# soedinglab/plass

Measured on AMD Instinct MI355X. Metric: read-overlaps/s per assembly iteration, higher is better.
Workload: dtype u8/u64 (integer hash, byte compare; f32 ratios)

## Files before the change

### plass_amd/csrc/assemble.hip

```cpp
#include "common.hpp"
#include "device_utils.hpp"
#include "posterior_class.hpp"
#include "ref_rules.hpp"
#include "asm_rules.hpp"
#include "host_util.hpp"
#include <algorithm>
#include <memory>
#include <cstring>

namespace plasship {

struct Item {
    uint32_t target; int32_t score; uint32_t alnLength; float seqId;
    int32_t qStart, qEnd; uint32_t qLen; int32_t dbStart, dbEnd; uint32_t dbLen;
    uint32_t state;
    uint32_t pad;
};

struct AsmArgs {
    SeqView s;
    const uint64_t *qoff; const AlnRec *recs;
    Item *items;
    const uint64_t *arenaOff;
    const uint32_t *leftCap;
    char *arena;
    uint32_t *flags;
    uint32_t *newLen;
    uint64_t *newStart;
    const signed char *mat;
    double lambda, logK, ln2;
    float seqIdThr; uint64_t maxSeqLen; int rescoreMode;
    uint32_t ownLaneMin;
    unsigned long long *stats;
    uint32_t *bigList; uint32_t nBig;
    const uint32_t *bigCount;
    uint32_t *overList; uint32_t *overCount;
    uint32_t queueCap;
    uint32_t *dbgRounds; uint32_t *dbgCycles;
    uint32_t *midList; uint32_t nMid;
    uint32_t *mid32List; uint32_t nMid32;
    uint32_t *smallList; uint32_t nSmall;
    uint32_t *narrowList; uint32_t nNarrow;
    uint32_t *heap;
    const uint32_t *ambKeys; const uint8_t *ambVals; uint32_t ambMask;
    uint32_t *needKeys; uint32_t *needCount; uint32_t needCap;
    uint32_t *redoList; uint32_t *redoCount;
    const uint32_t *queryList; uint32_t nQueryList;
    uint8_t *cmpCache;
    SeqView aa; char *aaArena; const uint64_t *aaArenaOff; const uint32_t *aaLeftCap; uint32_t *aaNewLen; uint64_t *aaNewStart;
};

__device__ __forceinline__ float seqIdThroughText(float f) {
    if (f == 1.0f) return 1.0f;
    const int t = (int) (f * 1000);
    int zeros = 0;
    if ((double) f < 0.10) zeros++;
    if ((double) f < 0.01) zeros++;
    int digits = 1; for (int x = t; x >= 10; x /= 10) digits++;
    double den = 1.0; for (int i = 0; i < digits + zeros; i++) den *= 10.0;
    return (float) ((double) t / den);
}

template <int G> __device__ __forceinline__ void copyBytesG(char *dst, const char *src, unsigned n, int gl) {
    for (unsigned i = 8u * (unsigned) gl; i < n; i += 8u * G) {
        const uint64_t w = loadU64Unaligned(src + i);
        if (i + 8 <= n) storeU64Unaligned(dst + i, w);
        else storeTail(dst + i, w, n - i);
    }
}
__device__ __forceinline__ void stageScoreTable(signed char *smat, const signed char *__restrict__ mat, int nThreads) {
    for (int i = threadIdx.x; i < 123 * 123; i += nThreads) smat[i] = i ? mat[i] : (signed char) 0;
}
__device__ __forceinline__ uint64_t byteRangeMask(int lo, int hi) {
    const uint64_t belowHi = hi >= 8 ? ~0ULL : (hi <= 0 ? 0ULL : ((1ULL << (8 * hi)) - 1ULL));
    const uint64_t belowLo = lo >= 8 ? ~0ULL : (lo <= 0 ? 0ULL : ((1ULL << (8 * lo)) - 1ULL));
    return belowHi & ~belowLo;
}
__device__ __forceinline__ int zeroBytesMasked(uint64_t x, uint64_t mask) {
    const uint64_t lo7 = 0x7F7F7F7F7F7F7F7FULL;
    return __popcll(~(((x & lo7) + lo7) | x | lo7) & mask);
}
template <int G> __device__ __forceinline__ void scoreColumnsG(const char *q, const char *t, unsigned len, const signed char *smat, int gl,
                                                               unsigned &first, unsigned &last, int &s, int &ids) {
    const unsigned p0 = 8u * (unsigned) gl;
    uint64_t qw = 0, tw = 0;
    if (p0 < len) { qw = loadU64Unaligned(q + p0); tw = loadU64Unaligned(t + p0); }
    const char q0 = q[0], t0 = t[0], qe = q[len - 1], te = t[len - 1];
    first = (q0 == '*' || t0 == '*') ? 1u : 0u;
    last = len - 1;
    if (last > 0 && (qe == '*' || te == '*')) last--;
    for (unsigned p = p0; p < len; p += 8u * G) {
        if (p != p0) { qw = loadU64Unaligned(q + p); tw = loadU64Unaligned(t + p); }
        const int lo = (int) first - (int) p, hi = (int) last - (int) p;
        uint64_t qv = qw, tv = tw;
        if (lo <= 0 && hi >= 8) ids += zeroBytesMasked(qw ^ tw, ~0ULL);
        else {
            const uint64_t m = byteRangeMask(lo, hi + 1);
            ids += zeroBytesMasked(qw ^ tw, byteRangeMask(lo, hi));
            qv = qw & m; tv = tw & m;
        }
#pragma unroll
        for (unsigned j = 0; j < 8; j++) {
// ... 911 lines not shown
        }
    }
    nExt = waveReduceSumU64(nExt); nResc = waveReduceSumU64(nResc); nRescRes = waveReduceSumU64(nRescRes); nAln = waveReduceSumU64(nAln); nQRes = waveReduceSumU64(nQRes);
    if (laneId() == 0) {
        if (nExt) atomicAdd(&a.stats[0], nExt); if (nResc) atomicAdd(&a.stats[1], nResc); if (nRescRes) atomicAdd(&a.stats[2], nRescRes);
        if (nAln) { atomicAdd(&a.stats[3], nAln); atomicAdd(&a.stats[4], nQRes); atomicAdd(&a.stats[5], nRescRes); }
    }
}

template <int G> __device__ __forceinline__ int groupSum(int v) {
    v = rowSum<(G < 16 ? G : 16)>(v);
#pragma unroll
    for (int o = 16; o < G; o <<= 1) v += __shfl_xor(v, o, G);
    return v;
}
template <int G> __device__ __forceinline__ unsigned long long groupMax(unsigned long long v) {
    v = rowMax<(G < 16 ? G : 16)>(v);
#pragma unroll
    for (int o = 16; o < G; o <<= 1) { const unsigned long long ok = __shfl_xor(v, o, G); v = (ok > v) ? ok : v; }
    return v;
}
template <int G> __device__ __forceinline__ uint32_t groupRank(uint32_t mine) {
    if (G == 8) return rowCountLess8(mine);
    uint32_t r = rowCountLess16(mine, mine, false);
#pragma unroll
    for (int o = 16; o < G; o += 16) r += rowCountLess16((uint32_t) __shfl_xor((int) mine, o, G), mine, true);
    return r;
}
template <int G> __device__ __forceinline__ unsigned long long groupBallot(bool p) {
    const unsigned long long m = __ballot(p);
    if (G == 64) return m;
    return (m >> ((laneId() / G) * G)) & ((1ULL << G) - 1ULL);
}

template <int G>
__device__ __forceinline__ Rescored rescoreOnDiagonalG(const char *q, unsigned qLen, const char *t, unsigned tLen, int diagonal,
                                                       const signed char *smat, int gl) {
    Rescored r; r.startPos = -1; r.endPos = -1; r.score = 0; r.diagonalLen = 0; r.idExcl = 0;
    const unsigned dist = (unsigned) abs(diagonal);
    unsigned qo, to, len;
    if (diagonal >= 0 && dist < qLen) { qo = dist; to = 0; len = min(tLen, qLen - dist); }
    else if (diagonal < 0 && dist < tLen) { qo = 0; to = dist; len = min(tLen - dist, qLen); }
    else return r;
    r.diagonalLen = len;
    if (len == 0) return r;
    unsigned first, last;
    int s = 0, ids = 0;
    scoreColumnsG<G>(q + qo, t + to, len, smat, gl, first, last, s, ids);
    s = groupSum<G>(s); ids = groupSum<G>(ids);
    r.score = (unsigned) max(s, 0); r.startPos = (int) first; r.endPos = (int) last; r.idExcl = ids;
    return r;
}

constexpr int ASM8_WPE = 5;
template <int G, int WPE>
__global__ __launch_bounds__(256) __attribute__((amdgpu_waves_per_eu(WPE, WPE))) void assembleGroupKernel(AsmArgs a) {
    __shared__ signed char smat[123 * 123 + 7];
    stageScoreTable(smat, a.mat, 256);
    __syncthreads();
    const int gl = threadIdx.x & (G - 1);
    const uint32_t groupsTotal = gridDim.x * (256 / G);
    const uint32_t nWork = (G == 64) ? a.nMid : ((G == 32) ? a.nMid32 : ((G == 16) ? a.nSmall : a.nNarrow));
    unsigned long long nExt = 0, nResc = 0, nRescRes = 0, nAln = 0, nQRes = 0;
    const uint32_t *workList = (G == 64) ? a.midList : ((G == 32) ? a.mid32List : ((G == 16) ? a.smallList : a.narrowList));
    auto loadWord = [&](uint32_t pid) -> uint64_t {
        uint64_t v = 0;
        if (pid != 0xFFFFFFFFu) {
            if (gl == 0) v = a.qoff[pid]; else if (gl == 1) v = a.qoff[pid + 1]; else if (gl == 2) v = a.arenaOff[pid]; else if (gl == 3) v = a.s.offLen[pid]; else if (gl == 4) v = a.leftCap[pid];
        }
        return v;
    };
    uint32_t w = blockIdx.x * (256 / G) + threadIdx.x / G;
    uint32_t idNext = (w < nWork) ? workList[w] : 0xFFFFFFFFu;
    uint64_t wordNext = loadWord(idNext);
    uint32_t idAhead = (w + groupsTotal < nWork) ? workList[w + groupsTotal] : 0xFFFFFFFFu;
    for (; w < nWork; w += groupsTotal) {
        const uint32_t id = idNext;
        const uint64_t h0 = __shfl(wordNext, 0, G), h1 = __shfl(wordNext, 1, G), aoff = __shfl(wordNext, 2, G), qOffLen = __shfl(wordNext, 3, G), qLeftCap = __shfl(wordNext, 4, G);
        idNext = idAhead; wordNext = loadWord(idNext);
        idAhead = (w + 2u * groupsTotal < nWork) ? workList[w + 2u * groupsTotal] : 0xFFFFFFFFu;
        const uint32_t h = (uint32_t) (h1 - h0);
        const char *orig = a.s.data + (qOffLen >> 24);
        unsigned querySeqLen = (unsigned) ((uint32_t) qOffLen & 0xFFFFFFu);
        if (gl == 0) { nAln += h; nQRes += querySeqLen; }
        uint32_t xTarget = 0xFFFFFFFFu, xAlnLen = 0, xQLen = 0, xDbLen = 0, xState = 2, xTLen = 0; uint64_t xTOff = 0;
        int xScore = 0, xQStart = 0, xQEnd = 0, xDbStart = 0, xDbEnd = 0;
        if ((uint32_t) gl < h) {
            const AlnRec r = a.recs[h0 + gl];
            xTarget = r.target;
            xAlnLen = (uint32_t) alnLengthOf(r.qStart, r.qEnd, r.dbStart, r.dbEnd);
            xScore = scorePerCol100(rawScoreOfBits(r.bitScore, a.ln2, a.logK, a.lambda), xAlnLen);
            xQStart = r.qStart; xQEnd = r.qEnd; xQLen = (uint32_t) r.qLen; xDbStart = r.dbStart; xDbEnd = r.dbEnd; xDbLen = (uint32_t) r.dbLen;
            xState = (xTarget == id || !r.accepted) ? 2u : 0u;
            const bool branchType = ((xDbStart == 0 && xDbEnd != (int) xDbLen - 1) || (xQStart == 0 && xQEnd != (int) xQLen - 1)) && !(xDbStart == 0 && xQStart == 0);
            if (xState == 0 && branchType) { xTOff = seqOff(a.s, xTarget); xTLen = seqLen(a.s, xTarget); }
        }
        const uint32_t tRank = groupRank<G>(xTarget);
        char *buf = a.arena + aoff;
        uint64_t curStart = qLeftCap;
        copyBytesG<G>(buf + curStart, orig, querySeqLen, gl);
        uint64_t curLen = querySeqLen;
        bool couldExtend = false;
        uint32_t inQueue = (uint32_t) __popcll(groupBallot<G>(xState == 0));
        while (inQueue > 0) {
            unsigned leftOff = 0, rightOff = 0;
            bool brokeOut = false;
            if (xState == 1) xState = 2;
            unsigned long long key = 0;
            bool rType = false, lType = false, rBranch = false, lBranch = false;
            unsigned fragR = 0;
            if (xState == 0) {
                key = ((unsigned long long) ((uint32_t) xScore ^ 0x80000000u) << 32) | ((unsigned long long) xAlnLen << 6) | (unsigned long long) (63u - tRank);
                if (isBranchType(xQStart, xQEnd, xQLen, xDbStart, xDbEnd, xDbLen)) {
                    if (xDbStart == 0) { rBranch = true; fragR = rightFragLen(xTLen, xDbEnd); rType = canExtendRight(fragR, xQEnd, querySeqLen); }
                    else if (xQStart == 0) { lBranch = true; lType = canExtendLeft(xDbStart, xDbEnd, xTLen); }
                }
            }
            const unsigned long long bestR = groupMax<G>(rType ? key : 0ULL), bestL = groupMax<G>(lType ? key : 0ULL);
            const bool rFirst = bestR != 0 && bestR > bestL;
            const bool isR = rType && key == bestR, isL = lType && key == bestL;
            auto extendRight = [&]() {
                const int bi = __ffsll((long long) groupBallot<G>(isR)) - 1;
                const char *tSeq = a.s.data + __shfl(xTOff, bi, G);
                const uint32_t bTarget = __shfl(xTarget, bi, G);
                const unsigned fragLen = __shfl(fragR, bi, G), dbEnd = (unsigned) __shfl(xDbEnd, bi, G);
                copyBytesG<G>(buf + curStart + curLen, tSeq + dbEnd + 1, fragLen, gl);
                curLen += fragLen; rightOff += fragLen;
                if (gl == 0) atomicOr(&a.flags[bTarget], 0x80u);
            };
            if (rFirst) extendRight();
            if (bestL != 0) {
                const int bi = __ffsll((long long) groupBallot<G>(isL)) - 1;
                const unsigned fragLen = (unsigned) __shfl(xDbStart, bi, G);
                if (curLen + fragLen >= a.maxSeqLen) brokeOut = true;
                else {
                    const char *tSeq = a.s.data + __shfl(xTOff, bi, G);
                    const uint32_t bTarget = __shfl(xTarget, bi, G);
                    curStart -= fragLen;
                    copyBytesG<G>(buf + curStart, tSeq, fragLen, gl);
                    curLen += fragLen; leftOff += fragLen;
                    if (gl == 0) atomicOr(&a.flags[bTarget], 0x80u);
                }
            }
            if (bestR != 0 && !rFirst && !brokeOut) extendRight();
            if (xState == 0 && (!brokeOut || key >= bestL)) {
                uint32_t st = 2;
                if (!(isR && (rFirst || !brokeOut)) && !isL) {
                    if (rBranch) { if (deferredRight(fragR, xQEnd, querySeqLen, rightOff)) st = 1; }
                    else if (lBranch) { if (deferredLeft(xDbStart, xDbEnd, xTLen, leftOff)) st = 1; }
                }
                xState = st;
            }
            inQueue = (uint32_t) __popcll(groupBallot<G>(xState == 0));
            if (leftOff > 0 || rightOff > 0) couldExtend = true;
            if (brokeOut && inQueue > 0) break;
            querySeqLen = (unsigned) curLen;
            const char *qs = buf + curStart;
            unsigned long long deferred = groupBallot<G>(xState == 1);
            if (deferred) waveMemSync();
            if (G >= 32 && (uint32_t) __popcll(deferred) >= a.ownLaneMin) {
                if (xState == 1) {
                    const char *tSeq = a.s.data + xTOff;
                    const int diag = (int) ((unsigned) xQStart + leftOff) - xDbStart;
                    const DiagSpan sp = diagonalSpan(diag, querySeqLen, xTLen);
                    unsigned first = 0, last = 0; int sc = 0, ids = 0; int startPos = -1, endPos = -1;
                    if (sp.hit && sp.len > 0) { scoreColumnsSerial(qs + sp.qo, tSeq + sp.to, sp.len, smat, first, last, sc, ids); startPos = (int) first; endPos = (int) last; }
                    const unsigned score = (unsigned) max(sc, 0);
                    nResc += 1; nRescRes += sp.len;
                    const AlnCoords c = alnOnDiagonal(diag, startPos, endPos);
                    xQLen = querySeqLen; xDbLen = xTLen; xAlnLen = sp.len; xScore = scorePerCol100(score, sp.len);
                    xQStart = c.qStart; xQEnd = c.qEnd; xDbStart = c.dbStart; xDbEnd = c.dbEnd;
                    xState = (rescoredSeqId(ids, c.qStart, c.qEnd) >= a.seqIdThr) ? 0u : 2u;
                }
                deferred = 0;
            }
            while (deferred) {
                const int dl = __ffsll((long long) deferred) - 1;
                deferred &= deferred - 1;
                const int dqs = __shfl(xQStart, dl, G), dds = __shfl(xDbStart, dl, G);
                const char *tSeq = a.s.data + __shfl(xTOff, dl, G);
                const unsigned tLen = __shfl(xTLen, dl, G);
                const int diag = (int) ((unsigned) dqs + leftOff) - dds;
                const Rescored rs = rescoreOnDiagonalG<G>(qs, querySeqLen, tSeq, tLen, diag, smat, gl);
                nResc += (gl == 0); nRescRes += (gl == 0) ? rs.diagonalLen : 0;
                const AlnCoords c = alnOnDiagonal(diag, rs.startPos, rs.endPos);
                const float seqId = rescoredSeqId(rs.idExcl, c.qStart, c.qEnd);
                if (gl == dl) {
                    xQLen = querySeqLen; xDbLen = tLen; xAlnLen = rs.diagonalLen; xScore = scorePerCol100(rs.score, rs.diagonalLen);
                    xQStart = c.qStart; xQEnd = c.qEnd; xDbStart = c.dbStart; xDbEnd = c.dbEnd;
                    xState = (seqId >= a.seqIdThr) ? 0u : 2u;
                }
            }
            inQueue = (uint32_t) __popcll(groupBallot<G>(xState == 0));
        }
        if (couldExtend) {
            if (gl == 0) { atomicOr(&a.flags[id], 0x20u); a.newLen[id] = (uint32_t) curLen; a.newStart[id] = aoff + curStart; nExt++; }
        }
    }
    nExt = waveReduceSumU64(nExt); nResc = waveReduceSumU64(nResc); nRescRes = waveReduceSumU64(nRescRes); nAln = waveReduceSumU64(nAln); nQRes = waveReduceSumU64(nQRes);
    if (laneId() == 0) {
        if (nExt) atomicAdd(&a.stats[0], nExt); if (nResc) atomicAdd(&a.stats[1], nResc); if (nRescRes) atomicAdd(&a.stats[2], nRescRes);
        const int tier = (G <= 16) ? 0 : 1;
        if (nAln) { atomicAdd(&a.stats[3 + 3 * tier], nAln); atomicAdd(&a.stats[4 + 3 * tier], nQRes); atomicAdd(&a.stats[5 + 3 * tier], nRescRes); }
    }
}

__global__ __launch_bounds__(256) void arenaSumKernel(const AlnRec *__restrict__ recs, uint64_t nAln, uint64_t maxSeqLen, unsigned long long *__restrict__ qSum,
                                                      unsigned long long *__restrict__ qSumAa, uint32_t *__restrict__ qCan, int mirror) {
    const int lane = laneId();
    for (uint64_t i = (uint64_t) blockIdx.x * blockDim.x + threadIdx.x; i < nAln; i += (uint64_t) gridDim.x * blockDim.x) {
        const AlnRec r = recs[i];
        const uint32_t id = r.query;
        uint32_t add = 0, addAa = 0; bool can = false;
        if (r.target != id && r.accepted) {
            add = (uint32_t) r.dbLen; addAa = (uint32_t) r.dbLen / 3 + 2;
            AlnCoords c; c.qStart = r.qStart; c.qEnd = r.qEnd; c.dbStart = r.dbStart; c.dbEnd = r.dbEnd;
            if (mirror && c.qStart > c.qEnd) c = mirrorReverseHit(r.qStart, r.qEnd, r.dbStart, r.dbEnd, (unsigned) r.dbLen);
            if (isBranchType(c.qStart, c.qEnd, (unsigned) r.qLen, c.dbStart, c.dbEnd, (unsigned) r.dbLen)) {
                if (c.dbStart == 0) can = canExtendRight(rightFragLen((unsigned) r.dbLen, c.dbEnd), c.qEnd, (unsigned) r.qLen);
                else if (c.qStart == 0) can = canExtendLeft(c.dbStart, c.dbEnd, (unsigned) r.dbLen) && ((uint64_t) r.qLen + (uint64_t) c.dbStart < maxSeqLen);
            }
        }
        const unsigned long long act = __ballot(1);
        const uint32_t prevId = (uint32_t) __shfl_up((int) id, 1, 64);
        const bool head = lane == 0 || prevId != id;
        const unsigned long long heads = __ballot(head), cans = __ballot(can);
        const int segStart = 63 - __clzll((long long) (heads & (lane == 63 ? ~0ULL : ((2ULL << lane) - 1ULL))));
        const unsigned long long later = lane == 63 ? 0ULL : (heads & ~((2ULL << lane) - 1ULL));
// ... 462 lines not shown
        (guided && (dAaLens.alloc((M + 1) * 8) != hipSuccess || dAaStart.alloc((M + 2) * 8) != hipSuccess))) { setError("plasship_assemble: out of device memory"); return PLASSHIP_ERR_DEVICE; }
    if (M) {
        const unsigned gridM = (unsigned) std::min<uint64_t>((M + 255) / 256, 8192);
        hipLaunchKernelGGL(extLensKernel, dim3(gridM), dim3(256), 0, st, gMeta.as<ExtMeta>(), M, dLens.as<uint64_t>(), guided ? dAaLens.as<uint64_t>() : (uint64_t *) nullptr);
        if (exclusiveScanU64(st, dLens.as<uint64_t>(), dStart.as<uint64_t>(), M, dTmp2.p, tmp2Bytes) ||
            (guided && exclusiveScanU64(st, dAaLens.as<uint64_t>(), dAaStart.as<uint64_t>(), M, dTmp2.p, tmp2Bytes))) { setError("plasship_assemble: scan failed"); return PLASSHIP_ERR_DEVICE; }
        hipLaunchKernelGGL(extMergeKernel, dim3(gridM), dim3(256), 0, st, gMeta.as<ExtMeta>(), M, dStart.as<uint64_t>(), guided ? dAaStart.as<uint64_t>() : (const uint64_t *) nullptr,
                           dFlags, dNewLen, dNewStart, dAaNewLen, dAaNewStart);
    }
    PH_TRACE(st, "assemble: merged the extended sequences");
    if (!keepTarget) {
        DevBuf gFlags;
        rc = commAllgathervBytes(ctx, dFlags, (uint64_t) N * 4, gFlags, rb); if (rc) return rc;
        if (N) hipLaunchKernelGGL(orFlagsKernel, dim3(gridN), dim3(256), 0, st, gFlags.as<uint32_t>(), N, W, dFlags);
        PH_CHECK(plasship::streamSync(st));
    }
    PH_CHECK(plasship::streamSync(st));
    PH_CHECK(hipGetLastError());
    return PLASSHIP_OK;
}

static bool asmHistOn() { return getenv("PLASSHIP_DEBUG_ASMHIST") != nullptr; }
static int asmHistRecord(hipStream_t st, uint32_t N, const uint64_t *dQoff, const uint32_t *dBigList, uint32_t nBig, const uint32_t *dRounds, const uint32_t *dCycles,
                         uint32_t cap, const uint32_t *tierQueries) {
    static int call = 0;
    std::vector<uint32_t> ids(nBig), rounds(N), cycles(N);
    std::vector<uint64_t> qoff((size_t) N + 1);
    if (nBig) PH_COPY_SYNC(st, ids.data(), dBigList, (size_t) nBig * 4, hipMemcpyDeviceToHost);
    PH_COPY_SYNC(st, qoff.data(), dQoff, ((size_t) N + 1) * 8, hipMemcpyDeviceToHost);
    PH_COPY_SYNC(st, rounds.data(), dRounds, (size_t) N * 4, hipMemcpyDeviceToHost);
    PH_COPY_SYNC(st, cycles.data(), dCycles, (size_t) N * 4, hipMemcpyDeviceToHost);
    constexpr int NH = 5, NR = 8;
    uint64_t hq[NH] = {}, hx[NH] = {}, hr[NH] = {}, hc[NH] = {}, hm[NH] = {}, rq[NR] = {}, ct = 0, over = 0, maxH = 0;
    for (uint32_t w = 0; w < nBig; w++) {
        const uint32_t id = ids[w], h = (uint32_t) (qoff[id + 1] - qoff[id]), r = rounds[id] & 0x7FFFFFFFu;
        int b = 0; while (b < NH - 1 && h > (128u << b)) b++;
        int k = 0; if (r) { k = 1; uint32_t e = 1; while (k < NR - 1 && r > e) { e <<= 1; k++; } }
        hq[b]++; hx[b] += rounds[id] >> 31; hr[b] += r; hm[b] = std::max<uint64_t>(hm[b], r); hc[b] += cycles[id]; ct += cycles[id];
        rq[k]++; over += h > cap; maxH = std::max<uint64_t>(maxH, h);
    }
    std::string s = "asmHist call " + std::to_string(call++) + " big queries " + std::to_string(nBig) + " (max h " + std::to_string(maxH) + ", over cap " +
                    std::to_string(cap) + ": " + std::to_string(over) + ") | h bins <=128,<=256,<=512,<=1024,more: queries/extended/mean rounds/max rounds/% ticks";
    for (int b = 0; b < NH; b++) {
        char t[96];
        snprintf(t, sizeof(t), " [%llu %llu %.2f %llu %.1f%%]", (unsigned long long) hq[b], (unsigned long long) hx[b], hq[b] ? (double) hr[b] / hq[b] : 0.0,
                 (unsigned long long) hm[b], ct ? 100.0 * hc[b] / ct : 0.0);
        s += t;
    }
    s += " | rounds 0,1,2,<=4,<=8,<=16,<=32,more:";
    for (int k = 0; k < NR; k++) s += " " + std::to_string(rq[k]);
    s += " | tier queries <=8,<=16,<=32,<=64,more:";
    for (int t = 0; t < 5; t++) s += " " + std::to_string(tierQueries[t]);
    fprintf(stderr, "%s\n", s.c_str());
    return PLASSHIP_OK;
}

static int assembleImpl(plasship_ctx *ctx, const plasship_seqdb *db, const plasship_seqdb *aaDb, const plasship_alns *al,
                        const plasship_assemble_params *par, plasship_seqdb **out, plasship_seqdb **outAa, plasship_assemble_stats *stats) {
    const bool guided = aaDb != nullptr;
    const bool nucl = db->dbtype == PLASSHIP_DBTYPE_NUCLEOTIDES;
    if (!nucl && db->dbtype != PLASSHIP_DBTYPE_AMINO_ACIDS) { setError("plasship_assemble: the sequence DB is neither amino acids nor nucleotides"); return PLASSHIP_ERR_ARG; }
    if (par->rescore_mode != 3) { setError("plasship_assemble: only --rescore-mode 3"); return PLASSHIP_ERR_UNSUPPORTED; }
    if (al->nQueries != db->n) { setError("plasship_assemble: alignment list does not belong to the DB"); return PLASSHIP_ERR_ARG; }
    PH_ENTER(ctx);
    hipStream_t st = ctx->stream;
    const uint32_t N = (uint32_t) db->n;
    if (nucl) { const int rcS = finishSelfAlns(ctx, al); if (rcS) return rcS; }
    const uint64_t nLines = al->nSlots;
    DevBuf dLeftCap, dBytes, dArenaOff, dTmp, dItems, dFlags, dNewLen, dNewStart, dMat, dStats, dArena;
    const size_t tmpBytes = exclusiveScanTmpBytes((size_t) N + 2);
    if (dLeftCap.alloc(((size_t) N + 1) * 4) != hipSuccess || dBytes.alloc(((size_t) N + 1) * 8) != hipSuccess || dArenaOff.alloc(((size_t) N + 2) * 8) != hipSuccess ||
        dTmp.alloc(tmpBytes) != hipSuccess || dItems.alloc(std::max<uint64_t>(nLines, 1) * sizeof(Item)) != hipSuccess || dFlags.alloc(((size_t) N + 1) * 4) != hipSuccess ||
        dNewLen.alloc(((size_t) N + 1) * 4) != hipSuccess || dNewStart.alloc(((size_t) N + 1) * 8) != hipSuccess || dMat.alloc(123 * 123) != hipSuccess || dStats.alloc(128) != hipSuccess) {
        setError("plasship_assemble: out of device memory"); return PLASSHIP_ERR_DEVICE;
    }
    PH_CHECK(hipMemsetAsync(dFlags.p, 0, ((size_t) N + 1) * 4, st));
    PH_CHECK(hipMemsetAsync(dNewLen.p, 0, ((size_t) N + 1) * 4, st));
    PH_CHECK(hipMemsetAsync(dStats.p, 0, 128, st));
    PH_CHECK(hipMemcpyAsync(dMat.p, asciiSubMat(nucl), 123 * 123, hipMemcpyHostToDevice, st));
    { const int rcOL = ensureOffLen(ctx, db); if (rcOL) return rcOL; }
    const SeqView sv = db->view();
    PH_CHECK(hipEventRecord(ctx->ev[0], st));
    const uint32_t nTiles = (uint32_t) (((size_t) N + SCAN_TILE - 1) / SCAN_TILE);
    DevBuf dBigList, dMidList, dMid32List, dSmallList, dNarrowList, dTierOf, dTierPart, dAaLeftCap, dAaBytes, dAaArenaOff, dAaArena, dAaNewLen, dAaNewStart;
    if (guided && (dAaLeftCap.alloc(((size_t) N + 1) * 4) != hipSuccess || dAaBytes.alloc(((size_t) N + 1) * 8) != hipSuccess || dAaArenaOff.alloc(((size_t) N + 2) * 8) != hipSuccess ||
                   dAaNewLen.alloc(((size_t) N + 1) * 4) != hipSuccess || dAaNewStart.alloc(((size_t) N + 1) * 8) != hipSuccess)) { setError("plasship_assemble: out of device memory"); return PLASSHIP_ERR_DEVICE; }
    if (guided) PH_CHECK(hipMemsetAsync(dAaNewLen.p, 0, ((size_t) N + 1) * 4, st));
    if (dBigList.alloc(((size_t) N + 1) * 4) != hipSuccess || dMidList.alloc(((size_t) N + 1) * 4) != hipSuccess || dMid32List.alloc(((size_t) N + 1) * 4) != hipSuccess ||
        dSmallList.alloc(((size_t) N + 1) * 4) != hipSuccess || (!nucl && dNarrowList.alloc(((size_t) N + 1) * 4) != hipSuccess) || dTierOf.alloc((size_t) N + 8) != hipSuccess ||
        dTierPart.alloc(((size_t) N_TIERS * (nTiles + 1) + 1) * 8) != hipSuccess) { setError("plasship_assemble: out of device memory"); return PLASSHIP_ERR_DEVICE; }
    DevBuf dQSum, dQSumAa, dQCan;
    if (dQSum.alloc(((size_t) N + 1) * 8) != hipSuccess || dQCan.alloc(((size_t) N + 1) * 4) != hipSuccess || (guided && dQSumAa.alloc(((size_t) N + 1) * 8) != hipSuccess)) { setError("plasship_assemble: out of device memory"); return PLASSHIP_ERR_DEVICE; }
    PH_CHECK(hipMemsetAsync(dQSum.p, 0, ((size_t) N + 1) * 8, st));
    PH_CHECK(hipMemsetAsync(dQCan.p, 0, ((size_t) N + 1) * 4, st));
    if (guided) PH_CHECK(hipMemsetAsync(dQSumAa.p, 0, ((size_t) N + 1) * 8, st));
    if (nLines) hipLaunchKernelGGL(arenaSumKernel, dim3((unsigned) std::min<uint64_t>((nLines + 255) / 256, (uint64_t) ctx->numCU * 32)), dim3(256), 0, st, al->d_recs.as<AlnRec>(), (uint64_t) nLines,
                                       (uint64_t) par->max_seq_len, dQSum.as<unsigned long long>(), guided ? dQSumAa.as<unsigned long long>() : (unsigned long long *) nullptr, dQCan.as<uint32_t>(),
                                       (nucl && !guided) ? 1 : 0);
    if (N) hipLaunchKernelGGL(arenaSizeKernel, dim3(std::min<uint32_t>((N + 255) / 256, 8192)), dim3(256), 0, st, sv, al->d_qoff.as<uint64_t>(), (const unsigned long long *) dQSum.as<unsigned long long>(),
                              (const unsigned long long *) dQSumAa.as<unsigned long long>(), (const uint32_t *) dQCan.as<uint32_t>(), dLeftCap.as<uint32_t>(), dBytes.as<uint64_t>(), nucl ? 1 : 0, (uint64_t) 1 << 30,
                              dTierOf.as<uint8_t>(),
                              guided ? aaDb->d_len.as<uint32_t>() : (const uint32_t *) nullptr, dAaLeftCap.as<uint32_t>(), guided ? dAaBytes.as<uint64_t>() : (uint64_t *) nullptr);
    if (guided && exclusiveScanU64(st, dAaBytes.as<uint64_t>(), dAaArenaOff.as<uint64_t>(), N, dTmp.p, tmpBytes)) { setError("plasship_assemble: scan failed"); return PLASSHIP_ERR_DEVICE; }
    PH_CHECK(hipMemsetAsync(dTierPart.p, 0, ((size_t) N_TIERS * (nTiles + 1) + 1) * 8, st));
    if (nTiles) hipLaunchKernelGGL(tierCountKernel, dim3(nTiles), dim3(SCAN_BLOCK), 0, st, (const uint8_t *) dTierOf.as<uint8_t>(), N, dTierPart.as<uint64_t>(), nTiles);
    if (exclusiveScanU64(st, dTierPart.as<uint64_t>(), dTierPart.as<uint64_t>(), (size_t) N_TIERS * (nTiles + 1), dTmp.p, tmpBytes)) { setError("plasship_assemble: scan failed"); return PLASSHIP_ERR_DEVICE; }
    {
        TierLists tl;
        tl.list[0] = dSmallList.as<uint32_t>(); tl.list[1] = dMid32List.as<uint32_t>(); tl.list[2] = dMidList.as<uint32_t>(); tl.list[3] = dBigList.as<uint32_t>();
        tl.list[TIER_NARROW] = dNarrowList.as<uint32_t>();
        if (nTiles) hipLaunchKernelGGL(tierListKernel, dim3(nTiles), dim3(SCAN_BLOCK), 0, st, (const uint8_t *) dTierOf.as<uint8_t>(), N, (const uint64_t *) dTierPart.as<uint64_t>(), nTiles, tl);
    }
    if (exclusiveScanU64(st, dBytes.as<uint64_t>(), dArenaOff.as<uint64_t>(), N, dTmp.p, tmpBytes)) { setError("plasship_assemble: scan failed"); return PLASSHIP_ERR_DEVICE; }
    uint64_t arenaBytes = 0, aaArenaBytes = 0;
    uint64_t rowStart[N_TIERS + 1] = {};
    if (guided) PH_CHECK(hipMemcpyAsync(&aaArenaBytes, dAaArenaOff.as<uint64_t>() + N, 8, hipMemcpyDeviceToHost, st));
    PH_CHECK(hipMemcpyAsync(&arenaBytes, dArenaOff.as<uint64_t>() + N, 8, hipMemcpyDeviceToHost, st));
    PH_CHECK(hipMemcpy2DAsync(rowStart, 8, dTierPart.p, (size_t) (nTiles + 1) * 8, 8, N_TIERS + 1, hipMemcpyDeviceToHost, st));
    PH_CHECK(plasship::streamSync(st));
    uint32_t cnts[N_TIERS];
    for (int t = 0; t < N_TIERS; t++) cnts[t] = (uint32_t) (rowStart[t + 1] - rowStart[t]);
    if (dArena.alloc(arenaBytes + 64) != hipSuccess || (guided && dAaArena.alloc(aaArenaBytes + 64) != hipSuccess)) {
        size_t fr = 0, tt = 0; (void) hipMemGetInfo(&fr, &tt);
        setError("plasship_assemble: out of device memory for the extension arena (" + std::to_string(arenaBytes) + " bytes; device free " + std::to_string(fr) + " of " + std::to_string(tt) + ")"); return PLASSHIP_ERR_DEVICE;
    }
    HostEvaluer ev(nucl, db->residues);
    AsmArgs a; memset(&a, 0, sizeof(a));
    a.s = sv; a.qoff = al->d_qoff.as<uint64_t>(); a.recs = al->d_recs.as<AlnRec>(); a.items = dItems.as<Item>(); a.arenaOff = dArenaOff.as<uint64_t>();
    a.leftCap = dLeftCap.as<uint32_t>(); a.arena = dArena.as<char>(); a.flags = dFlags.as<uint32_t>(); a.newLen = dNewLen.as<uint32_t>(); a.newStart = dNewStart.as<uint64_t>();
    a.mat = dMat.as<signed char>(); a.lambda = ev.g[0]; a.logK = ev.logK; a.ln2 = ev.ln2; a.seqIdThr = par->seq_id_thr; a.maxSeqLen = par->max_seq_len; a.rescoreMode = par->rescore_mode;
    a.ownLaneMin = 6;
    a.stats = dStats.as<unsigned long long>();
    a.smallList = dSmallList.as<uint32_t>(); a.nSmall = cnts[0];
    a.narrowList = dNarrowList.as<uint32_t>(); a.nNarrow = cnts[TIER_NARROW];
    a.mid32List = dMid32List.as<uint32_t>(); a.nMid32 = cnts[1];
    a.midList = dMidList.as<uint32_t>(); a.nMid = cnts[2];
    a.bigList = dBigList.as<uint32_t>(); a.nBig = cnts[3];
    if (!nucl && a.nBig) { const int rcS = finishSelfAlns(ctx, al, dBigList.as<uint32_t>(), a.nBig); if (rcS) return rcS; }
    std::unique_ptr<plasship_seqdb> aaPacked;
    if (guided && !aaDb->contiguous) {
        const int rcP = packedCopyOf(ctx, aaDb, aaPacked); if (rcP) return rcP;
    }
    if (guided) {
        a.aa = (aaPacked ? aaPacked.get() : aaDb)->view(); a.aaArena = dAaArena.as<char>(); a.aaArenaOff = dAaArenaOff.as<uint64_t>(); a.aaLeftCap = dAaLeftCap.as<uint32_t>();
        a.aaNewLen = dAaNewLen.as<uint32_t>(); a.aaNewStart = dAaNewStart.as<uint64_t>();
    }
    DevBuf dHeap, dNeed, dRedo[2], dCnt;
    if (nucl) {
        const uint32_t needCap = 1u << 16;
        if (dHeap.alloc(std::max<uint64_t>(nLines, 1) * 12) != hipSuccess || dNeed.alloc((size_t) needCap * 16) != hipSuccess || dRedo[0].alloc(((size_t) N + 1) * 4) != hipSuccess ||
            dRedo[1].alloc(((size_t) N + 1) * 4) != hipSuccess || dCnt.alloc(8) != hipSuccess) { setError("plasship_assemble: out of device memory"); return PLASSHIP_ERR_DEVICE; }
        a.heap = dHeap.as<uint32_t>();
        if (!ctx->d_cmpCache.p) {
            const size_t cb = (size_t) CMP_LEN * CMP_MM * CMP_LEN * CMP_MM;
            if (ctx->d_cmpCache.alloc(cb) != hipSuccess) { setError("plasship_assemble: out of device memory"); return PLASSHIP_ERR_DEVICE; }
            PH_CHECK(hipMemsetAsync(ctx->d_cmpCache.p, 0, cb, st));
        }
        a.cmpCache = ctx->d_cmpCache.as<uint8_t>();
        a.needKeys = dNeed.as<uint32_t>(); a.needCount = dCnt.as<uint32_t>(); a.needCap = needCap; a.redoCount = dCnt.as<uint32_t>() + 1;
        PH_CHECK(hipEventRecord(ctx->ev[2], st));
        uint32_t nWork = cnts[0] + cnts[1];
        for (int pass = 0; nWork > 0; pass++) {
            if (pass > 256) { setError("plasship_assemble: comparator table did not converge"); return PLASSHIP_ERR_DEVICE; }
            a.ambKeys = ctx->d_ambKeys.as<uint32_t>(); a.ambVals = ctx->d_ambVals.as<uint8_t>(); a.ambMask = ctx->ambSlots ? ctx->ambSlots - 1 : 0;
            a.redoList = dRedo[pass & 1].as<uint32_t>();
            PH_CHECK(hipMemsetAsync(dCnt.p, 0, 8, st));
            auto launchWave = [&](const uint32_t *list, uint32_t n) {
                if (!n) return;
                a.queryList = list; a.nQueryList = n;
                if (guided) hipLaunchKernelGGL(assembleNuclKernel<true>, dim3(std::min<uint32_t>(n, (uint32_t) ctx->numCU * 16)), dim3(64), 0, st, a);
                else hipLaunchKernelGGL(assembleNuclKernel<false>, dim3(std::min<uint32_t>(n, (uint32_t) ctx->numCU * 16)), dim3(64), 0, st, a);
            };
            if (pass == 0) {
                if (cnts[0]) {
                    DevBuf dCls;
                    if (dCls.alloc(2 * NW_CLASSES * 4) != hipSuccess) { setError("plasship_assemble: out of device memory"); return PLASSHIP_ERR_DEVICE; }
                    PH_CHECK(hipMemsetAsync(dCls.p, 0, 2 * NW_CLASSES * 4, st));
                    const unsigned g = std::min<uint32_t>((cnts[0] + 255) / 256, (uint32_t) ctx->numCU * 8);
                    hipLaunchKernelGGL(nuclClassCountKernel, dim3(g), dim3(256), 0, st, (const uint32_t *) dSmallList.as<uint32_t>(), cnts[0], (const uint64_t *) dBytes.as<uint64_t>(), dCls.as<uint32_t>());
                    hipLaunchKernelGGL(nuclClassScatterKernel, dim3(g), dim3(256), 0, st, (const uint32_t *) dSmallList.as<uint32_t>(), cnts[0], (const uint64_t *) dBytes.as<uint64_t>(), dCls.as<uint32_t>(),
                                       dMidList.as<uint32_t>());
                    a.queryList = dMidList.as<uint32_t>(); a.nQueryList = cnts[0];
                    const uint32_t grid = std::min<uint32_t>((cnts[0] + NT_BLOCK - 1) / NT_BLOCK, (uint32_t) ctx->numCU * 8);
                    if (guided) hipLaunchKernelGGL(assembleNuclThreadKernel<true>, dim3(grid), dim3(NT_BLOCK), 0, st, a);
                    else hipLaunchKernelGGL(assembleNuclThreadKernel<false>, dim3(grid), dim3(NT_BLOCK), 0, st, a);
                }
                launchWave(dMid32List.as<uint32_t>(), cnts[1]);
            } else launchWave(dRedo[(pass + 1) & 1].as<uint32_t>(), nWork);
            uint32_t cnt[2] = {0, 0};
            PH_CHECK(hipMemcpyAsync(cnt, dCnt.p, 8, hipMemcpyDeviceToHost, st));
            PH_CHECK(plasship::streamSync(st));
            PH_CHECK(hipGetLastError());
            nWork = cnt[1];
            if (nWork == 0) break;
            const uint32_t nNeed = std::min(cnt[0], needCap);
            if (nNeed == 0) { setError("plasship_assemble: queries aborted without a missing comparator tuple"); return PLASSHIP_ERR_DEVICE; }
            std::vector<uint32_t> need((size_t) nNeed * 4);
            PH_COPY_SYNC(ctx->stream, need.data(), dNeed.p, need.size() * 4, hipMemcpyDeviceToHost);
            const int rc = ambTableInsert(ctx, need.data(), nNeed);
            if (rc != PLASSHIP_OK) return rc;
        }
        PH_CHECK(hipEventRecord(ctx->ev[3], st));
        for (int e = 4; e <= 7; e++) PH_CHECK(hipEventRecord(ctx->ev[e], st));
    } else {
    const dim3 g16(std::min<uint32_t>((a.nSmall + 15) / 16, (uint32_t) ctx->numCU * 5u)), g64(std::min<uint32_t>((a.nMid + 3) / 4, (uint32_t) ctx->numCU * 4u));
    PH_CHECK(hipEventRecord(ctx->ev[2], st));
    if (a.nNarrow) hipLaunchKernelGGL((assembleGroupKernel<8, ASM8_WPE>), dim3(std::min<uint32_t>((a.nNarrow + 31) / 32, (uint32_t) ctx->numCU * ASM8_WPE)), dim3(256), 0, st, a);
    if (a.nSmall) hipLaunchKernelGGL((assembleGroupKernel<16, 5>), g16, dim3(256), 0, st, a);
    PH_CHECK(hipEventRecord(ctx->ev[3], st));
    PH_CHECK(hipEventRecord(ctx->ev[4], st));
    if (a.nMid32) hipLaunchKernelGGL((assembleGroupKernel<32, 5>), dim3(std::min<uint32_t>((a.nMid32 + 7) / 8, (uint32_t) ctx->numCU * 5u)), dim3(256), 0, st, a);
    if (a.nMid) hipLaunchKernelGGL((assembleGroupKernel<64, 4>), g64, dim3(256), 0, st, a);
    PH_CHECK(hipEventRecord(ctx->ev[5], st));
    PH_CHECK(hipEventRecord(ctx->ev[6], st));
    DevBuf dDbgRounds, dDbgCycles;
    const bool hist = asmHistOn();
    const uint32_t tierQ[5] = {a.nNarrow, a.nSmall, a.nMid32, a.nMid, a.nBig};
    if (hist) {
        if (dDbgRounds.alloc(((size_t) N + 1) * 4) != hipSuccess || dDbgCycles.alloc(((size_t) N + 1) * 4) != hipSuccess) { setError("plasship_assemble: out of device memory"); return PLASSHIP_ERR_DEVICE; }
        PH_CHECK(hipMemsetAsync(dDbgRounds.p, 0, ((size_t) N + 1) * 4, st));
        PH_CHECK(hipMemsetAsync(dDbgCycles.p, 0, ((size_t) N + 1) * 4, st));
        a.dbgRounds = dDbgRounds.as<uint32_t>(); a.dbgCycles = dDbgCycles.as<uint32_t>();
    }
    const bool onChip = tuneInt("ASMQ", 1) != 2;
    const uint32_t qCap = (uint32_t) std::max(0, std::min(tuneInt("ASMQ_CAP", (int) ASMQ_CAP), (int) ASMQ_CAP));
    const dim3 gBig(std::min<uint32_t>((a.nBig + 3) / 4, (uint32_t) ctx->numCU * 4u));
    DevBuf dOverList[2], dOverCount;
    if (a.nBig && onChip) {
        if (dOverList[0].alloc(((size_t) a.nBig + 1) * 4) != hipSuccess || dOverList[1].alloc(((size_t) a.nBig + 1) * 4) != hipSuccess || dOverCount.alloc(8) != hipSuccess) {
            setError("plasship_assemble: out of device memory"); return PLASSHIP_ERR_DEVICE;
        }
        PH_CHECK(hipMemsetAsync(dOverCount.p, 0, 8, st));
        AsmArgs q1 = a; q1.overList = dOverList[0].as<uint32_t>(); q1.overCount = dOverCount.as<uint32_t>(); q1.queueCap = qCap;
        hipLaunchKernelGGL((assembleQueueKernel<ASMQ_CAP1, 4>), dim3(std::min<uint32_t>((a.nBig + 3) / 4, (uint32_t) ctx->numCU * 4u)), dim3(256), 0, st, q1);
        AsmArgs q2 = q1; q2.bigList = dOverList[0].as<uint32_t>(); q2.bigCount = dOverCount.as<uint32_t>(); q2.overList = dOverList[1].as<uint32_t>(); q2.overCount = dOverCount.as<uint32_t>() + 1;
        hipLaunchKernelGGL((assembleQueueKernel<ASMQ_CAP, 2>), dim3(std::min<uint32_t>((a.nBig + 3) / 4, (uint32_t) ctx->numCU * 2u)), dim3(256), 0, st, q2);
        AsmArgs o = a; o.bigList = dOverList[1].as<uint32_t>(); o.bigCount = dOverCount.as<uint32_t>() + 1;
        hipLaunchKernelGGL(assembleBigKernel, gBig, dim3(256), 0, st, o);
    } else if (a.nBig) hipLaunchKernelGGL(assembleBigKernel, gBig, dim3(256), 0, st, a);
    PH_CHECK(hipEventRecord(ctx->ev[7], st));
    if (hist) { const int rcH = asmHistRecord(st, N, a.qoff, a.bigList, a.nBig, a.dbgRounds, a.dbgCycles, onChip ? qCap : 64, tierQ); if (rcH) return rcH; }
    }
    PH_TRACE(st, "assemble: extension kernels");
    plasship_seqdb *o = nullptr, *oAa = nullptr;
    unsigned long long hs[16] = {0};
    DevBuf dGathered, dGatheredAa;
    const char *arenaP = dArena.as<char>(), *aaArenaP = dAaArena.as<char>();
    if (commOf(ctx)) {
        const int rc = mergeExtended(ctx, N, guided, par->keep_target, dFlags.as<uint32_t>(), dNewLen.as<uint32_t>(), dNewStart.as<uint64_t>(), dArena.as<char>(),
                                     dAaNewLen.as<uint32_t>(), dAaNewStart.as<uint64_t>(), dAaArena.as<char>(), dTmp.p, tmpBytes, dGathered, dGatheredAa);
        if (rc != PLASSHIP_OK) return rc;
        arenaP = dGathered.as<char>(); aaArenaP = dGatheredAa.as<char>();
    }
    int rcOut = buildOutputDB(ctx, db, dFlags.as<uint32_t>(), dNewLen.as<uint32_t>(), dNewStart.as<uint64_t>(), arenaP, par->keep_target, dTmp.p, tmpBytes, &o,
                              dStats.p, hs, 128, guided ? (hipEvent_t) nullptr : ctx->ev[1], guided);
    if (rcOut != PLASSHIP_OK) return rcOut;
    std::unique_ptr<plasship_seqdb> holdO(o), holdAa;
    if (guided) {
        rcOut = buildOutputDB(ctx, aaDb, dFlags.as<uint32_t>(), dAaNewLen.as<uint32_t>(), dAaNewStart.as<uint64_t>(), aaArenaP, par->keep_target, dTmp.p, tmpBytes, &oAa,
                              nullptr, nullptr, 0, nullptr, true);
        if (rcOut != PLASSHIP_OK) return rcOut;
        holdAa.reset(oAa);
    }
    if (guided) { PH_CHECK(hipEventRecord(ctx->ev[1], st)); PH_CHECK(plasship::streamSync(st)); }
    if (hs[12]) { setError("plasship_guided_assemble: an alignment asks for a protein fragment the twin does not have (coordinates are not codon aligned)"); return PLASSHIP_ERR_ARG; }
    if (stats) {
// ... 35 lines not shown
```

Baseline: 780.1 million.

## Rescore deferred hits in eight-lane subgroups instead of serial or whole-group passes

For 32- and 64-lane groups, the deferred rescoring loop now splits the group into 8-lane subgroups. Each subgroup rescores one deferred hit in parallel, and the results are shuffled back to the owning lanes. This replaces both the per-lane serial path (used when many hits were deferred) and the one-hit-at-a-time whole-group path. The aim is to raise lane utilisation when several hits are deferred, at the cost of narrower per-hit parallelism on long diagonals. It also adds an optional env-gated histogram of deferred counts and overlap lengths.

```diff
diff --git a/plass_amd/csrc/assemble.hip b/plass_amd/csrc/assemble.hip
--- a/plass_amd/csrc/assemble.hip
+++ b/plass_amd/csrc/assemble.hip
@@ -30,7 +30,6 @@
     const signed char *mat;
     double lambda, logK, ln2;
     float seqIdThr; uint64_t maxSeqLen; int rescoreMode;
-    uint32_t ownLaneMin;
     unsigned long long *stats;
     uint32_t *bigList; uint32_t nBig;
     const uint32_t *bigCount;
@@ -48,6 +47,7 @@
     const uint32_t *queryList; uint32_t nQueryList;
     uint8_t *cmpCache;
     SeqView aa; char *aaArena; const uint64_t *aaArenaOff; const uint32_t *aaLeftCap; uint32_t *aaNewLen; uint64_t *aaNewStart;
+    unsigned long long *dbgDefer;
 };
 
 __device__ __forceinline__ float seqIdThroughText(float f) {
@@ -1065,6 +1065,10 @@
     return r;
 }
 
+constexpr int DEFER_OV = 65, DEFER_OV_BINS = 34, DEFER_PATH = DEFER_OV + DEFER_OV_BINS, DEFER_WORDS = DEFER_PATH + 2;
+__device__ __forceinline__ void deferHist(unsigned long long *h, int G, unsigned slot, unsigned long long v) { atomicAdd(&h[(G == 64 ? DEFER_WORDS : 0) + slot], v); }
+__device__ __forceinline__ unsigned deferOvBin(unsigned len) { return DEFER_OV + min((len + 15u) / 16u, (unsigned) DEFER_OV_BINS - 1u); }
+
 constexpr int ASM8_WPE = 5;
 template <int G, int WPE>
 __global__ __launch_bounds__(256) __attribute__((amdgpu_waves_per_eu(WPE, WPE))) void assembleGroupKernel(AsmArgs a) {
@@ -1171,22 +1175,44 @@
             const char *qs = buf + curStart;
             unsigned long long deferred = groupBallot<G>(xState == 1);
             if (deferred) waveMemSync();
-            if (G >= 32 && (uint32_t) __popcll(deferred) >= a.ownLaneMin) {
-                if (xState == 1) {
-                    const char *tSeq = a.s.data + xTOff;
-                    const int diag = (int) ((unsigned) xQStart + leftOff) - xDbStart;
-                    const DiagSpan sp = diagonalSpan(diag, querySeqLen, xTLen);
-                    unsigned first = 0, last = 0; int sc = 0, ids = 0; int startPos = -1, endPos = -1;
-                    if (sp.hit && sp.len > 0) { scoreColumnsSerial(qs + sp.qo, tSeq + sp.to, sp.len, smat, first, last, sc, ids); startPos = (int) first; endPos = (int) last; }
-                    const unsigned score = (unsigned) max(sc, 0);
-                    nResc += 1; nRescRes += sp.len;
-                    const AlnCoords c = alnOnDiagonal(diag, startPos, endPos);
-                    xQLen = querySeqLen; xDbLen = xTLen; xAlnLen = sp.len; xScore = scorePerCol100(score, sp.len);
-                    xQStart = c.qStart; xQEnd = c.qEnd; xDbStart = c.dbStart; xDbEnd = c.dbEnd;
-                    xState = (rescoredSeqId(ids, c.qStart, c.qEnd) >= a.seqIdThr) ? 0u : 2u;
-                }
-                deferred = 0;
-            }
+            if (G >= 32 && a.dbgDefer && gl == 0) {
+                const unsigned d = (unsigned) __popcll(deferred);
+                deferHist(a.dbgDefer, G, d, 1); deferHist(a.dbgDefer, G, DEFER_PATH, (d + G / 8 - 1) / (G / 8)); deferHist(a.dbgDefer, G, DEFER_PATH + 1, d);
+            }
+            if constexpr (G >= 32) {
+                constexpr int NB = G / 8;
+                const int sg = gl >> 3, sl = gl & 7;
+                while (deferred) {
+                    unsigned long long m = deferred;
+#pragma unroll
+                    for (int k = 0; k < NB - 1; k++) if (k < sg) m &= m - 1;
+                    const bool have = m != 0;
+                    const int dl = have ? __ffsll((long long) m) - 1 : gl;
+                    const int dqs = __shfl(xQStart, dl, G), dds = __shfl(xDbStart, dl, G);
+                    const char *tSeq = a.s.data + __shfl(xTOff, dl, G);
+                    const unsigned tLen = __shfl(xTLen, dl, G);
+                    int hScore = 0; unsigned hLen = 0, hPos = 0;
+                    if (have) {
+                        const int diag = (int) ((unsigned) dqs + leftOff) - dds;
+                        const Rescored rs = rescoreOnDiagonalG<8>(qs, querySeqLen, tSeq, tLen, diag, smat, sl);
+                        const AlnCoords c = alnOnDiagonal(diag, rs.startPos, rs.endPos);
+                        hScore = scorePerCol100(rs.score, rs.diagonalLen); hLen = rs.diagonalLen;
+                        hPos = ((unsigned) (rs.endPos + 1) << 3) | ((unsigned) (rs.startPos + 1) << 1) | (rescoredSeqId(rs.idExcl, c.qStart, c.qEnd) >= a.seqIdThr ? 1u : 0u);
+                    }
+                    const int rank = __popcll(deferred & ((1ULL << gl) - 1ULL)), src = 8 * (rank & (NB - 1));
+                    hScore = __shfl(hScore, src, G); hLen = __shfl(hLen, src, G); hPos = __shfl(hPos, src, G);
+                    if (((deferred >> gl) & 1ULL) && rank < NB) {
+                        nResc += 1; nRescRes += hLen;
+                        if (a.dbgDefer) deferHist(a.dbgDefer, G, deferOvBin(hLen), 1);
+                        const AlnCoords c = alnOnDiagonal((int) ((unsigned) xQStart + leftOff) - xDbStart, (int) ((hPos >> 1) & 3u) - 1, (int) (hPos >> 3) - 1);
+                        xQLen = querySeqLen; xDbLen = xTLen; xAlnLen = hLen; xScore = hScore;
+                        xQStart = c.qStart; xQEnd = c.qEnd; xDbStart = c.dbStart; xDbEnd = c.dbEnd;
+                        xState = (hPos & 1u) ? 0u : 2u;
+                    }
+#pragma unroll
+                    for (int k = 0; k < NB; k++) deferred &= deferred - 1;
+                }
+            } else
             while (deferred) {
                 const int dl = __ffsll((long long) deferred) - 1;
                 deferred &= deferred - 1;
@@ -1755,6 +1781,27 @@
     s += " | tier queries <=8,<=16,<=32,<=64,more:";
     for (int t = 0; t < 5; t++) s += " " + std::to_string(tierQueries[t]);
     fprintf(stderr, "%s\n", s.c_str());
+    return PLASSHIP_OK;
+}
+
+static bool asmDeferOn() { return getenv("PLASSHIP_DEBUG_ASMDEFER") != nullptr; }
+static int asmDeferRecord(hipStream_t st, const unsigned long long *dDefer) {
+    static int call = 0;
+    static unsigned long long tot[2 * DEFER_WORDS] = {};
+    unsigned long long h[2 * DEFER_WORDS];
+    PH_COPY_SYNC(st, h, dDefer, sizeof(h), hipMemcpyDeviceToHost);
+    for (int i = 0; i < 2 * DEFER_WORDS; i++) tot[i] += h[i];
+    call++;
+    for (int t = 0; t < 2; t++) {
+        const unsigned long long *c = tot + t * DEFER_WORDS;
+        std::string s = "asmDefer calls " + std::to_string(call) + " lanes " + std::to_string(t ? 64 : 32) + " | rounds by deferred hits 0,1,2,...:";
+        int last = 64; while (last > 0 && !c[last]) last--;
+        for (int d = 0; d <= last; d++) s += " " + std::to_string(c[d]);
+        s += " | re-scored hits by overlap columns 0,<=16,<=32,...,more than " + std::to_string(16 * (DEFER_OV_BINS - 2)) + ":";
+        for (int b = 0; b < DEFER_OV_BINS; b++) s += " " + std::to_string(c[DEFER_OV + b]);
+        s += " | eight-lane batches/hits " + std::to_string(c[DEFER_PATH]) + " " + std::to_string(c[DEFER_PATH + 1]);
+        fprintf(stderr, "%s\n", s.c_str());
+    }
     return PLASSHIP_OK;
 }
 
@@ -1832,7 +1879,6 @@
     a.s = sv; a.qoff = al->d_qoff.as<uint64_t>(); a.recs = al->d_recs.as<AlnRec>(); a.items = dItems.as<Item>(); a.arenaOff = dArenaOff.as<uint64_t>();
     a.leftCap = dLeftCap.as<uint32_t>(); a.arena = dArena.as<char>(); a.flags = dFlags.as<uint32_t>(); a.newLen = dNewLen.as<uint32_t>(); a.newStart = dNewStart.as<uint64_t>();
     a.mat = dMat.as<signed char>(); a.lambda = ev.g[0]; a.logK = ev.logK; a.ln2 = ev.ln2; a.seqIdThr = par->seq_id_thr; a.maxSeqLen = par->max_seq_len; a.rescoreMode = par->rescore_mode;
-    a.ownLaneMin = 6;
     a.stats = dStats.as<unsigned long long>();
     a.smallList = dSmallList.as<uint32_t>(); a.nSmall = cnts[0];
     a.narrowList = dNarrowList.as<uint32_t>(); a.nNarrow = cnts[TIER_NARROW];
@@ -1907,6 +1953,12 @@
         for (int e = 4; e <= 7; e++) PH_CHECK(hipEventRecord(ctx->ev[e], st));
     } else {
     const dim3 g16(std::min<uint32_t>((a.nSmall + 15) / 16, (uint32_t) ctx->numCU * 5u)), g64(std::min<uint32_t>((a.nMid + 3) / 4, (uint32_t) ctx->numCU * 4u));
+    DevBuf dDbgDefer;
+    if (asmDeferOn()) {
+        if (dDbgDefer.alloc(2 * DEFER_WORDS * 8) != hipSuccess) { setError("plasship_assemble: out of device memory"); return PLASSHIP_ERR_DEVICE; }
+        PH_CHECK(hipMemsetAsync(dDbgDefer.p, 0, 2 * DEFER_WORDS * 8, st));
+        a.dbgDefer = dDbgDefer.as<unsigned long long>();
+    }
     PH_CHECK(hipEventRecord(ctx->ev[2], st));
     if (a.nNarrow) hipLaunchKernelGGL((assembleGroupKernel<8, ASM8_WPE>), dim3(std::min<uint32_t>((a.nNarrow + 31) / 32, (uint32_t) ctx->numCU * ASM8_WPE)), dim3(256), 0, st, a);
     if (a.nSmall) hipLaunchKernelGGL((assembleGroupKernel<16, 5>), g16, dim3(256), 0, st, a);
@@ -1915,6 +1967,7 @@
     if (a.nMid32) hipLaunchKernelGGL((assembleGroupKernel<32, 5>), dim3(std::min<uint32_t>((a.nMid32 + 7) / 8, (uint32_t) ctx->numCU * 5u)), dim3(256), 0, st, a);
     if (a.nMid) hipLaunchKernelGGL((assembleGroupKernel<64, 4>), g64, dim3(256), 0, st, a);
     PH_CHECK(hipEventRecord(ctx->ev[5], st));
+    if (a.dbgDefer) { const int rcD = asmDeferRecord(st, a.dbgDefer); if (rcD) return rcD; }
     PH_CHECK(hipEventRecord(ctx->ev[6], st));
     DevBuf dDbgRounds, dDbgCycles;
     const bool hist = asmHistOn();
```

Result: no change. 786.5 million, median of 6 (+0.8%).
